# maxjaritz/mvpnet

Hardware: AMD Instinct MI355X
Metric: chunks/sec (8192 pts, 3x160x120 views) fwd+bwd (higher is better)
Workload: dtype f32; 1 GPU; configs[2]: MVPNet lifting (unproject + pixel k-NN + gather) + FeatureAggregation + PN2SSG full train step (fwd+loss+bwd+Adam), 2D CNN replaced by a resident 64-ch feature map; cfg=mvpnet_3d_unet_resnet34_pn2ssg.yaml, chunks_per_gpu=32, points=8192, views=3x160x120, feature_channels=64, k=3, parallelism=dp1 (one process per GPU, 1 grad all-reduce/step), launch=eager, cpu_affinity=32 logical cpus of 256 (0 .. 183)

## Files before the change

mvpnet_amd/csrc/mlp_stream.hip:

```cpp
#include "mlp_common.h"
#include "stats_reduce.h"
#include <algorithm>

namespace {

constexpr int kST = 256;
constexpr int kSLd = 36;

struct StreamArgs {
  const float* X;
  int64_t R;
  int Cin, ldx;
  const float* W;
  int ldw, Cout;
  InAct act;
  const float* bias;
  float* Y;
  double* partial;
  double* stat;
  int finalize;
  BnFinalize fin;
  int64_t tiles_per_wg;
  float* ymax;
  float* ymin;
  uint8_t* amax;
  uint8_t* amin;
};

template <int KS, int NB, bool ACT, int NS, bool POOL>
__global__ __launch_bounds__(kST) void mlp_stream_fwd_kernel(StreamArgs p) {
  using SP = SplitPairs<NS>;
  constexpr int kCols = NB * 32;
  constexpr int kWBytes = KS * NS * kCols * 64;
  __shared__ __attribute__((aligned(16))) unsigned char Wl[kWBytes];
  __shared__ __attribute__((aligned(16))) float Ps[4][KS * 32];
  __shared__ __attribute__((aligned(16))) float tiles[4][32 * kSLd];
  __shared__ double sred[2][4][kCols];
  const int tid = threadIdx.x, lane = tid & 63, wave = tid >> 6;
  const int li = lane & 31, lh = lane >> 5;
  const int Cin = p.Cin, Cout = p.Cout;

  for (int t = tid; t < kCols * KS * 8; t += kST) {
    const int co = t % kCols, kqi = t / kCols;
    const int k = 4 * kqi;
    float v[4];
#pragma unroll
    for (int e = 0; e < 4; ++e) v[e] = (co < Cout && k + e < Cin) ? p.W[(size_t)co * p.ldw + k + e] : 0.f;
    unsigned lo[NS], hi[NS];
    split_pair<NS>(v[0], v[1], lo);
    split_pair<NS>(v[2], v[3], hi);
    const int slab = kqi >> 3, kq = (kqi & 7) * 4;
    const int tt = kq >> 3, hh = (kq >> 2) & 1;
    const int unit = 2 * (tt >> 1) + hh, half = tt & 1;
#pragma unroll
    for (int pc = 0; pc < NS; ++pc)
      *reinterpret_cast<uint2*>(Wl + ((size_t)(slab * NS + pc) * kCols + co) * 64 + ((unit ^ ((co >> 2) & 3)) * 16) + half * 8) = make_uint2(lo[pc], hi[pc]);
  }
  if constexpr (ACT) {
    for (int k = tid; k < KS * 32; k += kST) {
      const int kc = min(k, Cin - 1);
      Ps[0][k] = p.act.mean[kc];
      Ps[1][k] = p.act.invstd[kc];
      Ps[2][k] = p.act.gamma[kc];
      Ps[3][k] = p.act.beta[kc];
    }
  }
  float bv[NB];
#pragma unroll
  for (int j = 0; j < NB; ++j) bv[j] = (p.bias && 32 * j + li < Cout) ? p.bias[32 * j + li] : 0.f;
  float ssum[NB], qsum[NB];
#pragma unroll
  for (int j = 0; j < NB; ++j) ssum[j] = qsum[j] = 0.f;
  __syncthreads();

  const int64_t ntiles = (p.R + 31) / 32;
  const int64_t t_begin = (int64_t)blockIdx.x * p.tiles_per_wg;
  const int64_t t_end = min(ntiles, t_begin + p.tiles_per_wg);
  float* st = tiles[wave];
  constexpr int PF = KS == 1 ? 3 : KS == 2 ? 2 : 1;
  float4 an[PF][KS][4];
  auto load_a = [&](float4 (&dst)[KS][4], int64_t t) {
    const int64_t row = min(t * 32 + li, p.R - 1);
    const float* xrow = p.X + (size_t)row * p.ldx;
#pragma unroll
    for (int sl = 0; sl < KS; ++sl)
#pragma unroll
      for (int tt = 0; tt < 4; ++tt) dst[sl][tt] = *reinterpret_cast<const float4*>(xrow + min(32 * sl + 8 * tt + 4 * lh, Cin - 4));
  };
#pragma unroll
  for (int u = 0; u < PF; ++u)
    if (t_begin + wave + 4 * u < t_end) load_a(an[u], t_begin + wave + 4 * u);
  for (int64_t tb = t_begin + wave; tb < t_end; tb += 4 * PF) {
#pragma unroll
   for (int u = 0; u < PF; ++u) {
    const int64_t t = tb + 4 * u;
    if (t >= t_end) break;
    float4 ac[KS][4];
#pragma unroll
    for (int sl = 0; sl < KS; ++sl)
#pragma unroll
      for (int tt = 0; tt < 4; ++tt) ac[sl][tt] = an[u][sl][tt];
    if (t + 4 * PF < t_end) load_a(an[u], t + 4 * PF);
    f32x16 acc[NB];
#pragma unroll
    for (int j = 0; j < NB; ++j)
#pragma unroll
      for (int i = 0; i < 16; ++i) acc[j][i] = 0.f;
#pragma unroll
    for (int sl = 0; sl < KS; ++sl) {
      float v[4][4];
#pragma unroll
      for (int tt = 0; tt < 4; ++tt) {
        v[tt][0] = ac[sl][tt].x; v[tt][1] = ac[sl][tt].y; v[tt][2] = ac[sl][tt].z; v[tt][3] = ac[sl][tt].w;
        if constexpr (ACT) {
          const int k = 32 * sl + 8 * tt + 4 * lh;
          const float4 m4 = *reinterpret_cast<const float4*>(&Ps[0][k]), i4 = *reinterpret_cast<const float4*>(&Ps[1][k]);
          const float4 g4 = *reinterpret_cast<const float4*>(&Ps[2][k]), b4 = *reinterpret_cast<const float4*>(&Ps[3][k]);
          const float pm[4] = {m4.x, m4.y, m4.z, m4.w}, pi[4] = {i4.x, i4.y, i4.z, i4.w};
          const float pg[4] = {g4.x, g4.y, g4.z, g4.w}, pb[4] = {b4.x, b4.y, b4.z, b4.w};
#pragma unroll
          for (int e = 0; e < 4; ++e) {
            const float a = ((v[tt][e] - pm[e]) * pi[e]) * pg[e] + pb[e];
            v[tt][e] = a > 0.f ? a : 0.f;
          }
        }
      }
#pragma unroll
      for (int s = 0; s < 2; ++s) {
        unsigned q0[NS], q1[NS], q2[NS], q3[NS];
        split_pair<NS>(v[2 * s][0], v[2 * s][1], q0);
        split_pair<NS>(v[2 * s][2], v[2 * s][3], q1);
        split_pair<NS>(v[2 * s + 1][0], v[2 * s + 1][1], q2);
        split_pair<NS>(v[2 * s + 1][2], v[2 * s + 1][3], q3);
        u32x4 af[NS];
#pragma unroll
        for (int pc = 0; pc < NS; ++pc) af[pc] = u32x4{q0[pc], q1[pc], q2[pc], q3[pc]};
        constexpr int JG = NB >= 2 ? 2 : 1;
#pragma unroll
        for (int j0 = 0; j0 < NB; j0 += JG) {
          u32x4 bfr[JG][NS];
#pragma unroll
          for (int jj = 0; jj < JG; ++jj) {
            const int co = 32 * (j0 + jj) + li;
#pragma unroll
            for (int pc = 0; pc < NS; ++pc)
              bfr[jj][pc] = *reinterpret_cast<const u32x4*>(Wl + ((size_t)(sl * NS + pc) * kCols + co) * 64 + (((2 * s + lh) ^ ((co >> 2) & 3)) * 16));
          }
#pragma unroll
          for (int qd = 0; qd < SP::N; ++qd)
#pragma unroll
            for (int jj = 0; jj < JG; ++jj)
              acc[j0 + jj] = __builtin_amdgcn_mfma_f32_32x32x16_bf16(__builtin_bit_cast(bf16x8, af[SP::A[qd]]),
                                                                     __builtin_bit_cast(bf16x8, bfr[jj][SP::B[qd]]), acc[j0 + jj], 0, 0, 0);
        }
      }
    }
    const int64_t r0 = t * 32;
#pragma unroll
    for (int j = 0; j < NB; ++j) {
      const bool cok = 32 * j + li < Cout;
      float s = 0.f, q = 0.f;
      if constexpr (POOL) {
        float vmax = -INFINITY, vmin = INFINITY;
        int rmax = 0, rmin = 0;
#pragma unroll
        for (int i = 0; i < 16; ++i) {
          const int m = (i & 3) + 8 * (i >> 2) + 4 * lh;
          const float y = acc[j][i] + bv[j];
          s += y;
          q += y * y;
          if (y > vmax) { vmax = y; rmax = m; }
          if (y < vmin) { vmin = y; rmin = m; }
        }
        const float omax = __shfl_xor(vmax, 32, kWave), omin = __shfl_xor(vmin, 32, kWave);
        const int ormax = __shfl_xor(rmax, 32, kWave), ormin = __shfl_xor(rmin, 32, kWave);
        if (omax > vmax || (omax == vmax && ormax < rmax)) { vmax = omax; rmax = ormax; }
        if (omin < vmin || (omin == vmin && ormin < rmin)) { vmin = omin; rmin = ormin; }
        if (lh == 0 && cok) {
          const size_t o = (size_t)t * Cout + 32 * j + li;
          p.ymax[o] = vmax;
          p.ymin[o] = vmin;
          p.amax[o] = (uint8_t)rmax;
          p.amin[o] = (uint8_t)rmin;
        }
        if (!cok) s = q = 0.f;
        ssum[j] += s;
        qsum[j] += q;
        continue;
      }
#pragma unroll
      for (int i = 0; i < 16; ++i) {
        const int m = (i & 3) + 8 * (i >> 2) + 4 * lh;
        float y = acc[j][i] + bv[j];
        y = (r0 + m < p.R && cok) ? y : 0.f;
        s += y;
        q += y * y;
        st[m * kSLd + li] = y;
      }
      ssum[j] += s;
      qsum[j] += q;
      __builtin_amdgcn_wave_barrier();
#pragma unroll
      for (int pp = 0; pp < 4; ++pp) {
        const int row = pp * 8 + (lane >> 3), c4 = (lane & 7) * 4;
        const f32x4 vv = *reinterpret_cast<const f32x4*>(st + row * kSLd + c4);
        const int64_t r = r0 + row;
        const int cc = 32 * j + c4;
        if (r < p.R && cc < Cout) __builtin_nontemporal_store(vv, reinterpret_cast<f32x4*>(p.Y + (size_t)r * Cout + cc));
      }
      __builtin_amdgcn_wave_barrier();
    }
   }
  }
  if (p.partial) {
#pragma unroll
    for (int j = 0; j < NB; ++j) {
      const float s = ssum[j] + __shfl_xor(ssum[j], 32, kWave), q = qsum[j] + __shfl_xor(qsum[j], 32, kWave);
      if (lane < 32) {
        sred[0][wave][32 * j + li] = (double)s;
        sred[1][wave][32 * j + li] = (double)q;
      }
    }
    __syncthreads();
    for (int col = tid; col < kCols; col += kST)
      if (col < Cout) {
        p.partial[((size_t)blockIdx.x * 2 + 0) * Cout + col] = sred[0][0][col] + sred[0][1][col] + sred[0][2][col] + sred[0][3][col];
        p.partial[((size_t)blockIdx.x * 2 + 1) * Cout + col] = sred[1][0][col] + sred[1][1][col] + sred[1][2][col] + sred[1][3][col];
      }
  } else if (p.stat) {
#pragma unroll
    for (int j = 0; j < NB; ++j) {
      const float s = ssum[j] + __shfl_xor(ssum[j], 32, kWave), q = qsum[j] + __shfl_xor(qsum[j], 32, kWave);
      if (lane < 32) {
        sred[0][wave][32 * j + li] = (double)s;
        sred[1][wave][32 * j + li] = (double)q;
      }
    }
    __syncthreads();
    for (int col = tid; col < kCols; col += kST)
      if (col < Cout) {
        atomicAdd(p.stat + col, sred[0][0][col] + sred[0][1][col] + sred[0][2][col] + sred[0][3][col]);
        atomicAdd(p.stat + Cout + col, sred[1][0][col] + sred[1][1][col] + sred[1][2][col] + sred[1][3][col]);
      }
    if (p.finalize) {
      __shared__ unsigned last;
      wait_vm_complete();
      __syncthreads();
      unsigned* ticket = reinterpret_cast<unsigned*>(p.stat + 2 * Cout);
      if (tid == 0) last = atomicAdd(ticket, 1u) == gridDim.x - 1 ? 1u : 0u;
      __syncthreads();
      if (!last) return;
      const BnFinalize& fin = p.fin;
      for (int c = tid; c < Cout; c += kST) {
        const double s1 = __hip_atomic_load(p.stat + c, __ATOMIC_RELAXED, __HIP_MEMORY_SCOPE_AGENT);
        const double s2 = __hip_atomic_load(p.stat + Cout + c, __ATOMIC_RELAXED, __HIP_MEMORY_SCOPE_AGENT);
        const double m = s1 / (double)fin.rows;
        double var = s2 / (double)fin.rows - m * m;
        if (var < 0.0) var = 0.0;
        fin.mean[c] = (float)m;
        fin.invstd[c] = (float)(1.0 / sqrt(var + (double)fin.eps));
        if (fin.running_mean) {
          const double unbiased = fin.rows > 1 ? var * ((double)fin.rows / (double)(fin.rows - 1)) : var;
          fin.running_mean[c] = (float)((1.0 - fin.momentum) * (double)fin.running_mean[c] + fin.momentum * m);
          fin.running_var[c] = (float)((1.0 - fin.momentum) * (double)fin.running_var[c] + fin.momentum * unbiased);
        }
      }
      if (tid == 0) {
        if (fin.num_batches_tracked) *fin.num_batches_tracked += 1;
        *ticket = 0u;
      }
    }
  }
}

template <int KS, int NB, int NS>
void launch_stream(const StreamArgs& a, unsigned grid, bool has_act, hipStream_t s) {
  if (a.ymax) {
    if (has_act) hipLaunchKernelGGL((mlp_stream_fwd_kernel<KS, NB, true, NS, true>), dim3(grid), dim3(kST), 0, s, a);
    else hipLaunchKernelGGL((mlp_stream_fwd_kernel<KS, NB, false, NS, true>), dim3(grid), dim3(kST), 0, s, a);
    return;
  }
  if (has_act) hipLaunchKernelGGL((mlp_stream_fwd_kernel<KS, NB, true, NS, false>), dim3(grid), dim3(kST), 0, s, a);
  else hipLaunchKernelGGL((mlp_stream_fwd_kernel<KS, NB, false, NS, false>), dim3(grid), dim3(kST), 0, s, a);
}

}

int mvp_mlp_stream_forward(const float* X, int64_t R, int Cin, int ldx, const float* W, int ldw, int Cout, const float* act_mean,
                           const float* act_invstd, const float* act_gamma, const float* act_beta, const float* bias, float* Y,
                           double* stat, double* partial, int ns, float bn_eps, float bn_momentum, float* bn_mean, float* bn_invstd,
                           float* bn_running_mean, float* bn_running_var, int64_t* bn_num_batches, float* ymax, float* ymin,
                           uint8_t* amax, uint8_t* amin, hipStream_t s) {
  const InAct act{act_mean, act_invstd, act_gamma, act_beta};
  if (ns == 0 || Cin > 128 || Cout > 128 || Cin < 4 || Cout % 4 != 0 || R < 32768 || (stat && !partial)) return MVP_EUNSUPPORTED;
  if (ldx % 4 != 0 || Cin % 4 != 0 || ((uintptr_t)X % 16) != 0 || (!ymax && ((uintptr_t)Y % 16) != 0)) return MVP_EUNSUPPORTED;
  if (ymax && R % 32 != 0) return MVP_EUNSUPPORTED;
  static const bool tail = []() { const char* e = getenv("MVP_STREAM_TAIL"); return !(e && e[0] == '0'); }();
  StreamArgs a{X, R, Cin, ldx, W, ldw, Cout, act, bias, Y, (stat && !tail) ? partial : nullptr, (stat && tail) ? stat : nullptr, bn_mean ? 1 : 0,
               BnFinalize{R, bn_eps, bn_momentum, bn_mean, bn_invstd, bn_running_mean, bn_running_var, bn_num_batches}, 0, ymax, ymin, amax, amin};
  const int64_t ntiles = cdiv(R, 32);
  const int ks = (int)cdiv(Cin, 32), nb = Cout <= 32 ? 1 : Cout <= 64 ? 2 : 4;
  const int64_t lds = (int64_t)ks * ns * nb * 32 * 64;
  const int64_t per_cu = std::max<int64_t>(1, std::min<int64_t>(4, (140 * 1024) / (lds + 24 * 1024)));
  int64_t wgs = std::min<int64_t>(256 * per_cu, std::min<int64_t>(cdiv(R, 128), cdiv(ntiles, 16)));
  wgs = std::max<int64_t>(wgs, 1);
  a.tiles_per_wg = cdiv(cdiv(ntiles, wgs), 4) * 4;
  const unsigned grid = (unsigned)cdiv(ntiles, a.tiles_per_wg);
  const bool has_act = act.mean != nullptr;
#define MVP_STREAM(KS_, NB_)                                                      \
  do {                                                                            \
    if (ns == 1) launch_stream<KS_, NB_, 1>(a, grid, has_act, s);                  \
    else if (ns == 2) launch_stream<KS_, NB_, 2>(a, grid, has_act, s);             \
    else launch_stream<KS_, NB_, 3>(a, grid, has_act, s);                          \
  } while (0)
#define MVP_STREAM_NB(KS_)                       \
  do {                                           \
    if (nb == 1) MVP_STREAM(KS_, 1);             \
    else if (nb == 2) MVP_STREAM(KS_, 2);        \
    else MVP_STREAM(KS_, 4);                     \
  } while (0)
  switch (ks) {
    case 1: MVP_STREAM_NB(1); break;
    case 2: MVP_STREAM_NB(2); break;
    case 3: MVP_STREAM_NB(3); break;
    default: MVP_STREAM_NB(4); break;
  }
#undef MVP_STREAM_NB
#undef MVP_STREAM
  int rc = mvp_launch_status();
  if (rc != MVP_OK) return rc;
  if (a.partial) {
    if (bn_mean)
      launch_stats_reduce_finalize(partial, (int64_t)grid, 2 * Cout, stat,
                                   BnFinalize{R, bn_eps, bn_momentum, bn_mean, bn_invstd, bn_running_mean, bn_running_var, bn_num_batches}, s);
    else
      launch_stats_reduce(partial, (int64_t)grid, 2 * Cout, stat, s);
  }
  return mvp_launch_status();
}
```

Baseline: 5167 chunks/s.

## Use 8-wave workgroups for large-weight stream MLP tiles with per-slab operand refill

Non-pooled stream-MLP instances whose LDS weight image exceeds 46 KiB now launch with 8 waves per workgroup instead of 4. This spreads the single copy of the weight image across more waves, so a CU has more concurrent waves when only one or two workgroups fit. In the 8-wave variant, activation prefetch is refilled slab by slab and LDS addresses are precomputed to hold down register pressure, with asm barriers steering codegen. Workgroups per CU now come from the HIP occupancy API rather than a hand-written LDS estimate, which may change grid sizing for every instance.

```diff
diff --git a/mvpnet_amd/csrc/mlp_stream.hip b/mvpnet_amd/csrc/mlp_stream.hip
--- a/mvpnet_amd/csrc/mlp_stream.hip
+++ b/mvpnet_amd/csrc/mlp_stream.hip
@@ -4,8 +4,14 @@
 
 namespace {
 
-constexpr int kST = 256;
 constexpr int kSLd = 36;
+
+constexpr int stream_waves(int ks, int nb, int ns, bool pool) { return (!pool && ks * ns * nb * 2048 > 46 * 1024) ? 8 : 4; }
+constexpr int64_t stream_lds_bytes(int ks, int nb, int ns, bool pool) {
+  const int w = stream_waves(ks, nb, ns, pool);
+  return (int64_t)ks * ns * nb * 2048 + 4 * ks * 32 * 4 + w * 32 * kSLd * 4 + 2 * w * nb * 32 * 8 + 16;
+}
+constexpr int64_t kLdsPerCu = 160 * 1024;
 
 struct StreamArgs {
   const float* X;
@@ -28,14 +34,16 @@
 };
 
 template <int KS, int NB, bool ACT, int NS, bool POOL>
-__global__ __launch_bounds__(kST) void mlp_stream_fwd_kernel(StreamArgs p) {
+__global__ __launch_bounds__(64 * stream_waves(KS, NB, NS, POOL), stream_waves(KS, NB, NS, POOL) / 4) void mlp_stream_fwd_kernel(StreamArgs p) {
   using SP = SplitPairs<NS>;
+  constexpr int kW = stream_waves(KS, NB, NS, POOL), kST = 64 * kW;
+  static_assert(stream_lds_bytes(KS, NB, NS, POOL) <= kLdsPerCu, "weight image + per-wave tiles + scratch exceed the CU's LDS");
   constexpr int kCols = NB * 32;
   constexpr int kWBytes = KS * NS * kCols * 64;
   __shared__ __attribute__((aligned(16))) unsigned char Wl[kWBytes];
   __shared__ __attribute__((aligned(16))) float Ps[4][KS * 32];
-  __shared__ __attribute__((aligned(16))) float tiles[4][32 * kSLd];
-  __shared__ double sred[2][4][kCols];
+  __shared__ __attribute__((aligned(16))) float tiles[kW][32 * kSLd];
+  __shared__ double sred[2][kW][kCols];
   const int tid = threadIdx.x, lane = tid & 63, wave = tid >> 6;
   const int li = lane & 31, lh = lane >> 5;
   const int Cin = p.Cin, Cout = p.Cout;
@@ -79,28 +87,49 @@
   float* st = tiles[wave];
   constexpr int PF = KS == 1 ? 3 : KS == 2 ? 2 : 1;
   float4 an[PF][KS][4];
-  auto load_a = [&](float4 (&dst)[KS][4], int64_t t) {
+  constexpr bool kSlabRefill = kW == 8;
+  unsigned wfrag[2][2];
+  if constexpr (kSlabRefill) {
+#pragma unroll
+    for (int s = 0; s < 2; ++s) {
+      wfrag[s][0] = (unsigned)(li * 64 + (((2 * s + lh) ^ ((li >> 2) & 3)) * 16));
+      wfrag[s][1] = wfrag[s][0] + 65536u;
+      asm volatile("" : "+v"(wfrag[s][1]));
+    }
+  }
+  auto load_slab = [&](float4 (&dst)[4], int64_t t, int sl) {
     const int64_t row = min(t * 32 + li, p.R - 1);
     const float* xrow = p.X + (size_t)row * p.ldx;
-#pragma unroll
-    for (int sl = 0; sl < KS; ++sl)
-#pragma unroll
-      for (int tt = 0; tt < 4; ++tt) dst[sl][tt] = *reinterpret_cast<const float4*>(xrow + min(32 * sl + 8 * tt + 4 * lh, Cin - 4));
+    int cmax = Cin - 4;
+    if constexpr (kSlabRefill) asm volatile("" : "+s"(cmax));
+#pragma unroll
+    for (int tt = 0; tt < 4; ++tt) {
+      const int k0 = 32 * sl + 8 * tt, col = k0 + 4 * lh;
+      if constexpr (kSlabRefill) dst[tt] = *reinterpret_cast<const float4*>(xrow + (sl < KS - 1 ? col : min(4 * lh, cmax - k0) + k0));
+      else dst[tt] = *reinterpret_cast<const float4*>(xrow + min(col, cmax));
+    }
   };
+  auto load_a = [&](float4 (&dst)[KS][4], int64_t t) {
+#pragma unroll
+    for (int sl = 0; sl < KS; ++sl) load_slab(dst[sl], t, sl);
+  };
 #pragma unroll
   for (int u = 0; u < PF; ++u)
-    if (t_begin + wave + 4 * u < t_end) load_a(an[u], t_begin + wave + 4 * u);
-  for (int64_t tb = t_begin + wave; tb < t_end; tb += 4 * PF) {
+    if (t_begin + wave + kW * u < t_end) load_a(an[u], t_begin + wave + kW * u);
+  for (int64_t tb = t_begin + wave; tb < t_end; tb += kW * PF) {
 #pragma unroll
    for (int u = 0; u < PF; ++u) {
-    const int64_t t = tb + 4 * u;
+    const int64_t t = tb + kW * u;
     if (t >= t_end) break;
-    float4 ac[KS][4];
-#pragma unroll
-    for (int sl = 0; sl < KS; ++sl)
-#pragma unroll
-      for (int tt = 0; tt < 4; ++tt) ac[sl][tt] = an[u][sl][tt];
-    if (t + 4 * PF < t_end) load_a(an[u], t + 4 * PF);
+    const bool more = t + kW * PF < t_end;
+    float4 ac[kSlabRefill ? 1 : KS][4];
+    if constexpr (!kSlabRefill) {
+#pragma unroll
+      for (int sl = 0; sl < KS; ++sl)
+#pragma unroll
+        for (int tt = 0; tt < 4; ++tt) ac[sl][tt] = an[u][sl][tt];
+      if (more) load_a(an[u], t + kW * PF);
+    }
     f32x16 acc[NB];
 #pragma unroll
     for (int j = 0; j < NB; ++j)
@@ -111,7 +140,13 @@
       float v[4][4];
 #pragma unroll
       for (int tt = 0; tt < 4; ++tt) {
-        v[tt][0] = ac[sl][tt].x; v[tt][1] = ac[sl][tt].y; v[tt][2] = ac[sl][tt].z; v[tt][3] = ac[sl][tt].w;
+        const float4 a4 = kSlabRefill ? an[u][sl][tt] : ac[kSlabRefill ? 0 : sl][tt];
+        v[tt][0] = a4.x; v[tt][1] = a4.y; v[tt][2] = a4.z; v[tt][3] = a4.w;
+      }
+      if constexpr (kSlabRefill)
+        if (more) load_slab(an[u][sl], t + kW * PF, sl);
+#pragma unroll
+      for (int tt = 0; tt < 4; ++tt) {
         if constexpr (ACT) {
           const int k = 32 * sl + 8 * tt + 4 * lh;
           const float4 m4 = *reinterpret_cast<const float4*>(&Ps[0][k]), i4 = *reinterpret_cast<const float4*>(&Ps[1][k]);
@@ -143,8 +178,14 @@
           for (int jj = 0; jj < JG; ++jj) {
             const int co = 32 * (j0 + jj) + li;
 #pragma unroll
-            for (int pc = 0; pc < NS; ++pc)
-              bfr[jj][pc] = *reinterpret_cast<const u32x4*>(Wl + ((size_t)(sl * NS + pc) * kCols + co) * 64 + (((2 * s + lh) ^ ((co >> 2) & 3)) * 16));
+            for (int pc = 0; pc < NS; ++pc) {
+              if constexpr (kSlabRefill) {
+                const unsigned c = (unsigned)(((sl * NS + pc) * kCols + 32 * (j0 + jj)) * 64);
+                bfr[jj][pc] = *reinterpret_cast<const u32x4*>(Wl + (c < 65536u ? wfrag[s][0] + c : wfrag[s][1] + (c - 65536u)));
+              } else {
+                bfr[jj][pc] = *reinterpret_cast<const u32x4*>(Wl + ((size_t)(sl * NS + pc) * kCols + co) * 64 + (((2 * s + lh) ^ ((co >> 2) & 3)) * 16));
+              }
+            }
           }
 #pragma unroll
           for (int qd = 0; qd < SP::N; ++qd)
@@ -156,6 +197,8 @@
       }
     }
     const int64_t r0 = t * 32;
+    int lrow = lane >> 3;
+    if constexpr (kSlabRefill) asm volatile("" : "+v"(lrow));
 #pragma unroll
     for (int j = 0; j < NB; ++j) {
       const bool cok = 32 * j + li < Cout;
@@ -202,7 +245,7 @@
       __builtin_amdgcn_wave_barrier();
 #pragma unroll
       for (int pp = 0; pp < 4; ++pp) {
-        const int row = pp * 8 + (lane >> 3), c4 = (lane & 7) * 4;
+        const int row = pp * 8 + lrow, c4 = (lane & 7) * 4;
         const f32x4 vv = *reinterpret_cast<const f32x4*>(st + row * kSLd + c4);
         const int64_t r = r0 + row;
         const int cc = 32 * j + c4;
@@ -212,6 +255,12 @@
     }
    }
   }
+  auto wave_sum = [](const double (&sr)[kW][kCols], int col) {
+    double v = sr[0][col];
+#pragma unroll
+    for (int w = 1; w < kW; ++w) v += sr[w][col];
+    return v;
+  };
   if (p.partial) {
 #pragma unroll
     for (int j = 0; j < NB; ++j) {
@@ -224,8 +273,8 @@
     __syncthreads();
     for (int col = tid; col < kCols; col += kST)
       if (col < Cout) {
-        p.partial[((size_t)blockIdx.x * 2 + 0) * Cout + col] = sred[0][0][col] + sred[0][1][col] + sred[0][2][col] + sred[0][3][col];
-        p.partial[((size_t)blockIdx.x * 2 + 1) * Cout + col] = sred[1][0][col] + sred[1][1][col] + sred[1][2][col] + sred[1][3][col];
+        p.partial[((size_t)blockIdx.x * 2 + 0) * Cout + col] = wave_sum(sred[0], col);
+        p.partial[((size_t)blockIdx.x * 2 + 1) * Cout + col] = wave_sum(sred[1], col);
       }
   } else if (p.stat) {
 #pragma unroll
@@ -239,8 +288,8 @@
     __syncthreads();
     for (int col = tid; col < kCols; col += kST)
       if (col < Cout) {
-        atomicAdd(p.stat + col, sred[0][0][col] + sred[0][1][col] + sred[0][2][col] + sred[0][3][col]);
-        atomicAdd(p.stat + Cout + col, sred[1][0][col] + sred[1][1][col] + sred[1][2][col] + sred[1][3][col]);
+        atomicAdd(p.stat + col, wave_sum(sred[0], col));
+        atomicAdd(p.stat + Cout + col, wave_sum(sred[1], col));
       }
     if (p.finalize) {
       __shared__ unsigned last;
@@ -273,15 +322,36 @@
   }
 }
 
+template <int KS, int NB, bool ACT, int NS, bool POOL>
+int stream_per_cu() {
+  static const int per_cu = []() {
+    int n = 0;
+    if (hipOccupancyMaxActiveBlocksPerMultiprocessor(&n, mlp_stream_fwd_kernel<KS, NB, ACT, NS, POOL>, 64 * stream_waves(KS, NB, NS, POOL), 0) != hipSuccess || n < 1) {
+      (void)hipGetLastError();
+      n = (int)(kLdsPerCu / stream_lds_bytes(KS, NB, NS, POOL));
+    }
+    return std::max(1, std::min(4, n));
+  }();
+  return per_cu;
+}
+
+template <int KS, int NB, bool ACT, int NS, bool POOL>
+unsigned launch_instance(StreamArgs a, hipStream_t s) {
+  constexpr int kW = stream_waves(KS, NB, NS, POOL);
+  const int64_t ntiles = cdiv(a.R, 32);
+  int64_t wgs = std::min<int64_t>(256 * stream_per_cu<KS, NB, ACT, NS, POOL>(), std::min<int64_t>(cdiv(a.R, 128), cdiv(ntiles, 16)));
+  wgs = std::max<int64_t>(wgs, 1);
+  a.tiles_per_wg = cdiv(cdiv(ntiles, wgs), kW) * kW;
+  const unsigned grid = (unsigned)cdiv(ntiles, a.tiles_per_wg);
+  hipLaunchKernelGGL((mlp_stream_fwd_kernel<KS, NB, ACT, NS, POOL>), dim3(grid), dim3(64 * kW), 0, s, a);
+  return grid;
+}
+
 template <int KS, int NB, int NS>
-void launch_stream(const StreamArgs& a, unsigned grid, bool has_act, hipStream_t s) {
-  if (a.ymax) {
-    if (has_act) hipLaunchKernelGGL((mlp_stream_fwd_kernel<KS, NB, true, NS, true>), dim3(grid), dim3(kST), 0, s, a);
-    else hipLaunchKernelGGL((mlp_stream_fwd_kernel<KS, NB, false, NS, true>), dim3(grid), dim3(kST), 0, s, a);
-    return;
-  }
-  if (has_act) hipLaunchKernelGGL((mlp_stream_fwd_kernel<KS, NB, true, NS, false>), dim3(grid), dim3(kST), 0, s, a);
-  else hipLaunchKernelGGL((mlp_stream_fwd_kernel<KS, NB, false, NS, false>), dim3(grid), dim3(kST), 0, s, a);
+unsigned launch_stream(const StreamArgs& a, bool has_act, hipStream_t s) {
+  if (a.ymax)
+    return has_act ? launch_instance<KS, NB, true, NS, true>(a, s) : launch_instance<KS, NB, false, NS, true>(a, s);
+  return has_act ? launch_instance<KS, NB, true, NS, false>(a, s) : launch_instance<KS, NB, false, NS, false>(a, s);
 }
 
 }
@@ -298,20 +368,14 @@
   static const bool tail = []() { const char* e = getenv("MVP_STREAM_TAIL"); return !(e && e[0] == '0'); }();
   StreamArgs a{X, R, Cin, ldx, W, ldw, Cout, act, bias, Y, (stat && !tail) ? partial : nullptr, (stat && tail) ? stat : nullptr, bn_mean ? 1 : 0,
                BnFinalize{R, bn_eps, bn_momentum, bn_mean, bn_invstd, bn_running_mean, bn_running_var, bn_num_batches}, 0, ymax, ymin, amax, amin};
-  const int64_t ntiles = cdiv(R, 32);
   const int ks = (int)cdiv(Cin, 32), nb = Cout <= 32 ? 1 : Cout <= 64 ? 2 : 4;
-  const int64_t lds = (int64_t)ks * ns * nb * 32 * 64;
-  const int64_t per_cu = std::max<int64_t>(1, std::min<int64_t>(4, (140 * 1024) / (lds + 24 * 1024)));
-  int64_t wgs = std::min<int64_t>(256 * per_cu, std::min<int64_t>(cdiv(R, 128), cdiv(ntiles, 16)));
-  wgs = std::max<int64_t>(wgs, 1);
-  a.tiles_per_wg = cdiv(cdiv(ntiles, wgs), 4) * 4;
-  const unsigned grid = (unsigned)cdiv(ntiles, a.tiles_per_wg);
+  unsigned grid = 0;
   const bool has_act = act.mean != nullptr;
 #define MVP_STREAM(KS_, NB_)                                                      \
   do {                                                                            \
-    if (ns == 1) launch_stream<KS_, NB_, 1>(a, grid, has_act, s);                  \
-    else if (ns == 2) launch_stream<KS_, NB_, 2>(a, grid, has_act, s);             \
-    else launch_stream<KS_, NB_, 3>(a, grid, has_act, s);                          \
+    if (ns == 1) grid = launch_stream<KS_, NB_, 1>(a, has_act, s);                 \
+    else if (ns == 2) grid = launch_stream<KS_, NB_, 2>(a, has_act, s);            \
+    else grid = launch_stream<KS_, NB_, 3>(a, has_act, s);                         \
   } while (0)
 #define MVP_STREAM_NB(KS_)                       \
   do {                                           \
```

Measured after the change: 5153 chunks/s. Within noise of the previous version (-0.3%).
